# Graph-COM/HEPT

Measured on AMD Instinct MI355X. Metric: attention-fwd points/sec, higher is better.
Workload: dtype bf16

## Files before the change

### hept_amd/csrc/block_attn.hip

```cpp
#include "common.h"
#include "p2p_dev.h"

namespace {

#ifndef HEPT_ATTN_STORE
#define HEPT_ATTN_STORE 1
#endif
__device__ __forceinline__ void store16_rows(unsigned int* dst, const u32x4& v) {
#if HEPT_ATTN_STORE == 1
    __builtin_nontemporal_store(v, reinterpret_cast<u32x4*>(dst));
#else
    *reinterpret_cast<u32x4*>(dst) = v;
#endif
}

#ifndef HEPT_RAGGED16_WAVES
#define HEPT_RAGGED16_WAVES 7
#endif
constexpr int attn_waves(int nkt, bool bf16, bool p16, bool full, bool diff = false) {
    if (diff) return full ? 3 : 2;
    return bf16 ? ((nkt == 3 && !p16 && full) ? 6 : (full ? 8 : HEPT_RAGGED16_WAVES)) : (full ? 6 : 4);
}
template <int NKT, bool BF16, bool P16, bool F16QK, bool FULL, bool DIFF = false>
__global__ __launch_bounds__(64 * NKT) __attribute__((amdgpu_waves_per_eu(attn_waves(NKT, BF16, P16, FULL, DIFF), attn_waves(NKT, BF16, P16, FULL, DIFF))))
void block_attn_kernel(const char* __restrict__ qhat,
                                                              const char* __restrict__ kvhat,
                                                              const int* __restrict__ qpos,
                                                              const int* __restrict__ kpos,
                                                              float* __restrict__ part, int N, int H, int D, int B,
                                                              int nb, HeadRange hr, PushArgs pa) {
    if (pa.push_wgs > 0 && (int)blockIdx.x < pa.push_wgs) {
        reduce_push_body<P16>(pa, (int)blockIdx.x);
        return;
    }
    constexpr int NT = 64 * NKT;
    constexpr int KEYS = 32 * NKT;
    constexpr int ESZ = BF16 ? 2 : 4;
    constexpr int QROW = 32 * ESZ;
    constexpr int KVROW = 2 * QROW;
    constexpr int CH = QROW / 16;
    constexpr int CPR = 2 * CH;

    extern __shared__ __attribute__((aligned(16))) char smem[];
    char* k_s = smem;
    char* v_s = smem + KEYS * QROW;
    float* kn_s = reinterpret_cast<float*>(smem + 2 * KEYS * QROW);
    int* qidx_s = reinterpret_cast<int*>(smem + 2 * KEYS * QROW + KEYS * 4);

    const int tid = threadIdx.x, lane = tid & 63, w = tid >> 6, hh = lane >> 5, li = lane & 31;
    const int bid = (int)blockIdx.x - pa.push_wgs;
    const int h = hr.h0 + bid % hr.hg;
    const int rest = bid / hr.hg;
    const int b = hr.tl > 0 ? rest / hr.tl : rest % nb, t = hr.tl > 0 ? rest % hr.tl : rest / nb;
    const size_t seg = ((size_t)t * H + h) * N + (size_t)b * B;
    const int* __restrict__ kp = kpos + seg;
    const int* __restrict__ qp = qpos + seg;
    const char* __restrict__ qbase = qhat + (size_t)h * N * QROW;
    const char* __restrict__ kvbase = kvhat + (size_t)h * N * KVROW;

    const int qi = w * 32 + li;
    const bool qvalid = FULL || qi < B;
    const int qsrc = qp[qvalid ? qi : 0];
    if (hh == 0) qidx_s[qi] = qvalid ? qsrc : -1;
    const char* qrow = qbase + (size_t)qsrc * QROW;
    float qn = *reinterpret_cast<const float*>(qrow + QROW - 4);
    u32x4 qraw[BF16 ? 2 : 4];
#pragma unroll
    for (int s = 0; s < (BF16 ? 2 : 4); ++s)
        qraw[s] = *reinterpret_cast<const u32x4*>(qrow + (BF16 ? (s * 32 + hh * 16) : (hh * 64 + s * 16)));
    if (hh == 1) qraw[BF16 ? 1 : 3][3] = 0u;
    if constexpr (DIFF) {
        static_assert(!BF16, "the difference form runs on f32 rows");
        float part = 0.f;
#pragma unroll
        for (int s2 = 0; s2 < 4; ++s2)
#pragma unroll
            for (int j = 0; j < 4; ++j) {
                const bool feat = 16 * hh + 4 * s2 + j < D;
                const float qv = __uint_as_float(qraw[s2][j]);
                part = feat ? fmaf(qv, qv, part) : part;
                if (!feat) qraw[s2][j] = 0u;
            }
        qn = -0.5f * (part + __shfl_xor(part, 32));
    }

#pragma unroll
    for (int it = 0; it < CPR / 2; ++it) {
        const int ci = it * NT + tid;
        const int key = ci / CPR, c = ci % CPR;
        u32x4 val = {0u, 0u, 0u, 0u};
        if (FULL || key < B) {
            const int src = kp[key];
            val = *reinterpret_cast<const u32x4*>(kvbase + (size_t)src * KVROW + c * 16);
        }
        if (c < CH) {
            if (c == CH - 1) {
                kn_s[key] = __uint_as_float(val[3]);
                val[3] = 0u;
            }
            const int sw = BF16 ? ((key >> 2) & 3) : ((key >> 1) & 7);
            *reinterpret_cast<u32x4*>(k_s + key * QROW + ((c ^ sw) * 16)) = val;
        } else {
            *reinterpret_cast<u32x4*>(v_s + key * QROW + (c - CH) * 16) = val;
        }
    }
    __syncthreads();
    if constexpr (DIFF) {
        if (tid < KEYS) {
            const int sw = (tid >> 1) & 7;
            float acc = 0.f;
            for (int col = 0; col < D; ++col) {
                const float kv2 = *reinterpret_cast<const float*>(k_s + tid * QROW + (((col >> 2) ^ sw) * 16) + (col & 3) * 4);
                acc = fmaf(kv2, kv2, acc);
            }
            kn_s[tid] = -0.5f * acc;
        }
        __syncthreads();
    }

    f32x16 z;
#pragma unroll
    for (int r = 0; r < 16; ++r) z[r] = 0.f;

#pragma unroll
    for (int kt = 0; kt < NKT; ++kt) {
        if (!FULL && kt * 32 >= B) break;
        const int key = kt * 32 + li;
        f32x16 x;
#pragma unroll
        for (int r = 0; r < 16; ++r) x[r] = qn + kn_s[kt * 32 + hept_acc_row(r, hh)];

        if constexpr (BF16) {
#pragma unroll
            for (int s = 0; s < 2; ++s) {
                const int c = 2 * s + hh;
                const u32x4 kraw =
                    *reinterpret_cast<const u32x4*>(k_s + key * QROW + ((c ^ ((key >> 2) & 3)) * 16));
                if constexpr (F16QK)
                    x = __builtin_amdgcn_mfma_f32_32x32x16_f16(__builtin_bit_cast(f16x8, kraw),
                                                               __builtin_bit_cast(f16x8, qraw[s]), x, 0, 0, 0);
                else
                    x = __builtin_amdgcn_mfma_f32_32x32x16_bf16(__builtin_bit_cast(bf16x8, kraw),
                                                                __builtin_bit_cast(bf16x8, qraw[s]), x, 0, 0, 0);
            }
        } else {
            float kf[16];
#pragma unroll
            for (int c = 0; c < 4; ++c) {
                const f32x4 kk = *reinterpret_cast<const f32x4*>(
                    k_s + key * QROW + (((4 * hh + c) ^ ((key >> 1) & 7)) * 16));
                kf[4 * c] = kk[0]; kf[4 * c + 1] = kk[1]; kf[4 * c + 2] = kk[2]; kf[4 * c + 3] = kk[3];
            }
#pragma unroll
            for (int s = 0; s < 16; ++s)
                x = __builtin_amdgcn_mfma_f32_32x32x2f32(kf[s], __uint_as_float(qraw[s >> 2][s & 3]), x, 0, 0, 0);
            if constexpr (DIFF) {
                float dsq[16];
#pragma unroll
                for (int r = 0; r < 16; ++r) dsq[r] = 0.f;
                for (int col = D; col < 30; ++col) {
                    const float qc = *reinterpret_cast<const float*>(qrow + col * 4);
#pragma unroll
                    for (int r = 0; r < 16; ++r) {
                        const int kr = kt * 32 + hept_acc_row(r, hh);
                        const float kc = *reinterpret_cast<const float*>(
                            k_s + kr * QROW + (((col >> 2) ^ ((kr >> 1) & 7)) * 16) + (col & 3) * 4);
                        const float dlt = qc - kc;
                        dsq[r] = fmaf(dlt, dlt, dsq[r]);
                    }
                }
#pragma unroll
                for (int r = 0; r < 16; ++r) x[r] = fmaf(-0.5f, dsq[r], x[r]);
            }
        }

        float pr[16];
        exp_clamped(x, pr);
        if (!FULL && (kt + 1) * 32 > B) {
#pragma unroll
            for (int r = 0; r < 16; ++r)
                if (kt * 32 + hept_acc_row(r, hh) >= B) pr[r] = 0.f;
        }

        if constexpr (BF16) {
            const int g = lane >> 4, l16 = lane & 15;
            const int vrow = kt * 32 + 4 * hh + (l16 >> 2);
            const int vcol = 32 * (g & 1) + 8 * (l16 & 3);
#pragma unroll
            for (int s = 0; s < 2; ++s) {
                u32x4 pw;
#pragma unroll
                for (int j = 0; j < 4; ++j) pw[j] = hept_pack_bf16(pr[8 * s + 2 * j], pr[8 * s + 2 * j + 1]);
                const s16x4 v0 = __builtin_amdgcn_ds_read_tr16_b64_v4i16(
                    (lds_s16x4_ptr)(v_s + (vrow + 16 * s) * QROW + vcol));
                const s16x4 v1 = __builtin_amdgcn_ds_read_tr16_b64_v4i16(
                    (lds_s16x4_ptr)(v_s + (vrow + 16 * s + 8) * QROW + vcol));
                typedef __attribute__((ext_vector_type(8))) short s16x8;
                const s16x8 vv = {v0[0], v0[1], v0[2], v0[3], v1[0], v1[1], v1[2], v1[3]};
                z = __builtin_amdgcn_mfma_f32_32x32x16_bf16(__builtin_bit_cast(bf16x8, pw),
                                                            __builtin_bit_cast(bf16x8, vv), z, 0, 0, 0);
            }
        } else {
#pragma unroll
            for (int r = 0; r < 16; ++r) {
                const float vv =
                    *reinterpret_cast<const float*>(v_s + (kt * 32 + hept_acc_row(r, hh)) * QROW + li * 4);
                z = __builtin_amdgcn_mfma_f32_32x32x2f32(pr[r], vv, z, 0, 0, 0);
            }
        }
    }

    if constexpr (P16) {
        __syncthreads();
        float* tile = reinterpret_cast<float*>(smem) + w * 32 * 32;
        {
            float* wr = tile + (4 * hh) * 32 + li;
#pragma unroll
            for (int r = 0; r < 16; ++r) wr[((r & 3) + 8 * (r >> 2)) * 32] = z[r];
        }
        unsigned int* __restrict__ pt =
            reinterpret_cast<unsigned int*>(part) + (size_t)t * hr.tstride_rows * 16 + (size_t)(h - hr.hsub) * 16;
#pragma unroll
        for (int j = 0; j < 2; ++j) {
            const int row = (lane >> 2) + 16 * j, pc = lane & 3;
            const int q2 = w * 32 + row;
            const f32x4 f0 = *reinterpret_cast<const f32x4*>(tile + row * 32 + pc * 8);
            const f32x4 f1 = *reinterpret_cast<const f32x4*>(tile + row * 32 + pc * 8 + 4);
            u32x4 v = {hept_pack_bf16(f0[0], f0[1]), hept_pack_bf16(f0[2], f0[3]), hept_pack_bf16(f1[0], f1[1]),
                       hept_pack_bf16(f1[2], f1[3])};
            if (pc == 3) v = u32x4{__float_as_uint(f0[0] + 1e-20f), 0u, 0u, 0u};
            if (FULL || q2 < B) {
                const int dst = qidx_s[q2];
                if (pa.direct) {
                    bool remote;
                    char* rowp = direct_row(pa, dst, h - hr.h0, 64, remote) + pc * 16;
                    if (remote) store16_system(rowp, v);
                    else *reinterpret_cast<u32x4*>(rowp) = v;
                } else {
                    store16_rows(pt + (size_t)dst * hr.hout * 16 + pc * 4, v);
                }
            }
        }
    } else {
        float* __restrict__ pt = part + (size_t)t * hr.tstride_rows * 32 + (size_t)(h - hr.hsub) * 32 + li;
#pragma unroll
        for (int r = 0; r < 16; ++r) {
            const int q2 = w * 32 + hept_acc_row(r, hh);
            if (FULL || q2 < B) {
                const int dst = qidx_s[q2];
                float val = z[r];
                if (li == D) val += 1e-20f;
                if (pa.direct) {
                    bool remote;
                    char* rowp = direct_row(pa, dst, h - hr.h0, 128, remote) + li * 4;
                    if (remote) store4_system(rowp, __float_as_uint(val));
                    else *reinterpret_cast<float*>(rowp) = val;
                } else {
                    pt[(size_t)dst * hr.hout * 32] = val;
                }
            }
        }
    }
    if (pa.direct) {
        drain_remote_stores();
        if (pa.counter) signal_when_all_done(pa.counter, pa.peers, pa.world, pa.flag_idx, pa.epoch, gridDim.x - pa.push_wgs);
    }
}

#ifndef HEPT_SPLIT_CK8
#define HEPT_SPLIT_CK8 128
#endif
constexpr int split_ck(int nkt) { return nkt == 8 ? HEPT_SPLIT_CK8 : (nkt >= 2 ? 64 : 32); }
#ifndef HEPT_SPLIT_PP
#define HEPT_SPLIT_PP 2
#endif
template <int NKT, bool FULL, int VP, bool DIFF = false>
__global__ __launch_bounds__(64 * NKT) void block_attn_split_kernel(const float* __restrict__ qhat,
                                                                    const float* __restrict__ kvhat,
                                                                    const int* __restrict__ qpos,
                                                                    const int* __restrict__ kpos,
                                                                    float* __restrict__ part, int N, int H, int D,
                                                                    int B, int nb, HeadRange hr, PushArgs pa) {
    if (pa.push_wgs > 0 && (int)blockIdx.x < pa.push_wgs) {
        reduce_push_body<false>(pa, (int)blockIdx.x);
        return;
    }
    constexpr int NT = 64 * NKT;
    constexpr int KEYS = 32 * NKT;
    constexpr int PROW = 64;
    constexpr int CK = split_ck(NKT);
    constexpr int NCH = (KEYS + CK - 1) / CK;
    constexpr int IPT = (CK * 8 + NT - 1) / NT;
    extern __shared__ __attribute__((aligned(16))) char smem[];
    char* k_s = smem;
    char* v_s = smem + 3 * CK * PROW;
    float* kc_s = reinterpret_cast<float*>(smem + (3 + VP) * CK * PROW);

    const int tid = threadIdx.x, lane = tid & 63, w = tid >> 6, hh = lane >> 5, li = lane & 31;
    const int bid = (int)blockIdx.x - pa.push_wgs;
    const int h = hr.h0 + bid % hr.hg;
    const int rest = bid / hr.hg;
    const int b = hr.tl > 0 ? rest / hr.tl : rest % nb, t = hr.tl > 0 ? rest % hr.tl : rest / nb;
    const size_t seg = ((size_t)t * H + h) * N + (size_t)b * B;
    const int* __restrict__ kp = kpos + seg;
    const int* __restrict__ qp = qpos + seg;
    const float* __restrict__ qbase = qhat + (size_t)h * N * 32;
    const float* __restrict__ kvbase = kvhat + (size_t)h * N * 64;

    float pre[IPT][8];
    auto fetch = [&](int ch) {
#pragma unroll
        for (int it = 0; it < IPT; ++it) {
            const int ci = it * NT + tid;
            const int key = ch * CK + (ci >> 3), c = ci & 7;
#pragma unroll
            for (int j = 0; j < 8; ++j) pre[it][j] = 0.f;
            if (ci < CK * 8 && key < (FULL ? KEYS : B)) {
                const int ks = kp[key];
                if (c >= 4 && hr.vsrc) {
                    const int col = 8 * (c - 4);
                    const float* src = hr.vsrc + ((size_t)ks * H + h) * D + col;
                    const bool real = ks < hr.raw_size;
                    if (real && col < D) {
                        const f32x4 a0 = *reinterpret_cast<const f32x4*>(src);
                        pre[it][0] = a0[0]; pre[it][1] = a0[1]; pre[it][2] = a0[2]; pre[it][3] = a0[3];
                    }
                    if (real && col + 4 < D) {
                        const f32x4 a1 = *reinterpret_cast<const f32x4*>(src + 4);
                        pre[it][4] = a1[0]; pre[it][5] = a1[1]; pre[it][6] = a1[2]; pre[it][7] = a1[3];
                    }
                    if (col == D) pre[it][0] = 1.f;
                    if (col + 4 == D) pre[it][4] = 1.f;
                } else {
                    const float* src = kvbase + (size_t)ks * 64 + c * 8;
                    const f32x4 a0 = *reinterpret_cast<const f32x4*>(src);
                    const f32x4 a1 = *reinterpret_cast<const f32x4*>(src + 4);
                    pre[it][0] = a0[0]; pre[it][1] = a0[1]; pre[it][2] = a0[2]; pre[it][3] = a0[3];
                    pre[it][4] = a1[0]; pre[it][5] = a1[1]; pre[it][6] = a1[2]; pre[it][7] = a1[3];
                    if (c == 3) pre[it][6] = 1.f;
                }
            }
        }
    };
    auto stage = [&]() {
#pragma unroll
        for (int it = 0; it < IPT; ++it) {
            const int ci = it * NT + tid;
            if (ci >= CK * 8) break;
            const int row = ci >> 3, c = ci & 7;
            u32x4 ph, pm, pl;
            if constexpr (DIFF) {
                float sq = 0.f;
                if (c < 3) {
#pragma unroll
                    for (int j = 0; j < 8; ++j) sq = fmaf(pre[it][j], pre[it][j], sq);
                }
                const int sqi = __builtin_bit_cast(int, sq);
                const float s1 = __builtin_bit_cast(float, __builtin_amdgcn_update_dpp(0, sqi, 0x111, 0xF, 0xF, true));
                const float s2 = __builtin_bit_cast(float, __builtin_amdgcn_update_dpp(0, sqi, 0x112, 0xF, 0xF, true));
                const float s3 = __builtin_bit_cast(float, __builtin_amdgcn_update_dpp(0, sqi, 0x113, 0xF, 0xF, true));
                if (c == 3) {
                    *reinterpret_cast<f32x4*>(kc_s + row * 8) = f32x4{pre[it][0], pre[it][1], pre[it][2], pre[it][3]};
                    *reinterpret_cast<f32x4*>(kc_s + row * 8 + 4) = f32x4{pre[it][4], pre[it][5], 0.f, 0.f};
#pragma unroll
                    for (int j = 0; j < 6; ++j) pre[it][j] = 0.f;
                    pre[it][7] = -0.5f * ((s3 + s2) + s1);
                }
            }
            if (c < 4) {
                split3_bf16(pre[it], ph, pm, pl);
                const int off = row * PROW + ((c ^ ((row >> 2) & 3)) * 16);
                *reinterpret_cast<u32x4*>(k_s + off) = ph;
                *reinterpret_cast<u32x4*>(k_s + CK * PROW + off) = pm;
                *reinterpret_cast<u32x4*>(k_s + 2 * CK * PROW + off) = pl;
            } else {
                if constexpr (VP == 3) split3_bf16(pre[it], ph, pm, pl);
                else split2_bf16(pre[it], ph, pm);
                const int off = row * PROW + (c - 4) * 16;
                *reinterpret_cast<u32x4*>(v_s + off) = ph;
                *reinterpret_cast<u32x4*>(v_s + CK * PROW + off) = pm;
                if constexpr (VP == 3) *reinterpret_cast<u32x4*>(v_s + 2 * CK * PROW + off) = pl;
            }
        }
    };
    fetch(0);

    const int qi = w * 32 + li;
    const bool qvalid = FULL || qi < B;
    const int qsrc = qp[qvalid ? qi : 0];
    const float* qrow = qbase + (size_t)qsrc * 32;
    u32x4 qh[2], qm[2], ql[2];
    float qc[DIFF ? 6 : 1];
    {
        float av[2][8];
#pragma unroll
        for (int s = 0; s < 2; ++s) {
            const f32x4 a0 = *reinterpret_cast<const f32x4*>(qrow + 16 * s + 8 * hh);
            const f32x4 a1 = *reinterpret_cast<const f32x4*>(qrow + 16 * s + 8 * hh + 4);
            av[s][0] = a0[0]; av[s][1] = a0[1]; av[s][2] = a0[2]; av[s][3] = a0[3];
            av[s][4] = a1[0]; av[s][5] = a1[1]; av[s][6] = a1[2]; av[s][7] = a1[3];
        }
        if constexpr (DIFF) {
            float fn = 0.f;
#pragma unroll
            for (int j = 0; j < 8; ++j) fn = fmaf(av[0][j], av[0][j], fn);
            if (hh == 0) {
#pragma unroll
                for (int j = 0; j < 8; ++j) fn = fmaf(av[1][j], av[1][j], fn);
            }
            fn += __shfl_xor(fn, 32);
#pragma unroll
            for (int c = 0; c < 6; ++c) qc[c] = __shfl(av[1][c], li + 32);
            if (hh == 1) {
#pragma unroll
                for (int j = 0; j < 6; ++j) av[1][j] = 0.f;
                av[1][6] = -0.5f * fn;
                av[1][7] = 1.f;
            }
        } else if (hh == 1) {
            av[1][6] = av[1][7];
            av[1][7] = 1.f;
        }
#pragma unroll
        for (int s = 0; s < 2; ++s) split3_bf16(av[s], qh[s], qm[s], ql[s]);
    }

    f32x16 z;
#pragma unroll
    for (int r = 0; r < 16; ++r) z[r] = 0.f;
    const int krow[2] = {li * PROW + ((hh ^ ((li >> 2) & 3)) * 16), li * PROW + (((2 + hh) ^ ((li >> 2) & 3)) * 16)};
    const int vlane = (4 * hh + ((lane & 15) >> 2)) * PROW + 32 * ((lane >> 4) & 1) + 8 * (lane & 3);

#pragma unroll
    for (int ch = 0; ch < NCH; ++ch) {
        if (!FULL && ch * CK >= B) break;
        if (ch > 0) __syncthreads();
        stage();
        if (ch + 1 < NCH) fetch(ch + 1);
        __syncthreads();
        constexpr int TPC = CK / 32, GRP = TPC < 2 ? TPC : 2;
#pragma unroll
        for (int g0 = 0; g0 < TPC; g0 += GRP) {
        f32x16 xs[GRP];
#pragma unroll
        for (int kg = 0; kg < GRP; ++kg) {
            const int kl = g0 + kg;
            const int kt = ch * TPC + kl;
            if (kt >= NKT) break;
            if (!FULL && kt * 32 >= B) break;
#pragma unroll
            for (int r = 0; r < 16; ++r) xs[kg][r] = 0.f;
#pragma unroll
            for (int s = 0; s < 2; ++s) {
                const int off = kl * 32 * PROW + krow[s];
                const u32x4 kh = *reinterpret_cast<const u32x4*>(k_s + off);
                const u32x4 km = *reinterpret_cast<const u32x4*>(k_s + CK * PROW + off);
                const u32x4 kl3 = *reinterpret_cast<const u32x4*>(k_s + 2 * CK * PROW + off);
                xs[kg] = mfma_bf16(kl3, qh[s], xs[kg]);
                xs[kg] = mfma_bf16(kh, ql[s], xs[kg]);
                xs[kg] = mfma_bf16(km, qm[s], xs[kg]);
                xs[kg] = mfma_bf16(km, qh[s], xs[kg]);
                xs[kg] = mfma_bf16(kh, qm[s], xs[kg]);
                xs[kg] = mfma_bf16(kh, qh[s], xs[kg]);
            }
        }
#pragma unroll
        for (int kg = 0; kg < GRP; ++kg) {
            const int kl = g0 + kg;
            const int kt = ch * TPC + kl;
            if (kt >= NKT) break;
            if (!FULL && kt * 32 >= B) break;
            f32x16 x = xs[kg];
            if constexpr (DIFF) {
#pragma unroll
                for (int r = 0; r < 16; ++r) {
                    const float* kc = kc_s + (kl * 32 + hept_acc_row(r, hh)) * 8;
                    const f32x4 k0 = *reinterpret_cast<const f32x4*>(kc), k1 = *reinterpret_cast<const f32x4*>(kc + 4);
                    float d0 = qc[0] - k0[0], d1 = qc[1] - k0[1], d2 = qc[2] - k0[2], d3 = qc[3] - k0[3];
                    float d4 = qc[4] - k1[0], d5 = qc[5] - k1[1];
                    float dsq = d0 * d0;
                    dsq = fmaf(d1, d1, dsq); dsq = fmaf(d2, d2, dsq); dsq = fmaf(d3, d3, dsq);
                    dsq = fmaf(d4, d4, dsq); dsq = fmaf(d5, d5, dsq);
                    x[r] = fmaf(-0.5f, dsq, x[r]);
                }
            }

            float pr[16];
            exp_clamped(x, pr);
            if (!FULL && (kt + 1) * 32 > B) {
#pragma unroll
                for (int r = 0; r < 16; ++r)
                    if (kt * 32 + hept_acc_row(r, hh) >= B) pr[r] = 0.f;
            }

#pragma unroll
            for (int s = 0; s < 2; ++s) {
                float pa[8];
#pragma unroll
                for (int j = 0; j < 8; ++j) pa[j] = pr[8 * s + j];
                constexpr int PP = HEPT_SPLIT_PP;
                u32x4 pp[3];
                if constexpr (PP == 3) split3_bf16(pa, pp[0], pp[1], pp[2]);
                else split2_bf16(pa, pp[0], pp[1]);
                typedef __attribute__((ext_vector_type(8))) short s16x8;
                u32x4 vpl[VP];
#pragma unroll
                for (int pl = 0; pl < VP; ++pl) {
                    const char* vb = v_s + pl * CK * PROW + (kl * 32 + 16 * s) * PROW + vlane;
                    const s16x4 v0 = __builtin_amdgcn_ds_read_tr16_b64_v4i16((lds_s16x4_ptr)(vb));
                    const s16x4 v1 = __builtin_amdgcn_ds_read_tr16_b64_v4i16((lds_s16x4_ptr)(vb + 8 * PROW));
                    const s16x8 vv = {v0[0], v0[1], v0[2], v0[3], v1[0], v1[1], v1[2], v1[3]};
                    vpl[pl] = __builtin_bit_cast(u32x4, vv);
                }
#pragma unroll
                for (int ord = 2; ord >= 0; --ord)
#pragma unroll
                    for (int i = PP - 1; i >= 0; --i) {
                        const int j = ord - i;
                        if (j >= 0 && j < VP) z = mfma_bf16(pp[i], vpl[j], z);
                    }
            }
        }
        }
    }

    __syncthreads();
    float* tile = reinterpret_cast<float*>(smem) + w * 32 * 32;
    {
        float* wr = tile + (4 * hh) * 32 + li;
#pragma unroll
        for (int r = 0; r < 16; ++r) wr[((r & 3) + 8 * (r >> 2)) * 32] = z[r];
    }
    float* __restrict__ pt = part + (size_t)t * hr.tstride_rows * 32 + (size_t)(h - hr.hsub) * 32;
#pragma unroll
    for (int j = 0; j < 4; ++j) {
        const int row = (lane >> 3) + 8 * j, pc = lane & 7;
        const int q2 = w * 32 + row;
        const int dst = __shfl(qsrc, row);
        f32x4 f = *reinterpret_cast<const f32x4*>(tile + row * 32 + pc * 4);
#pragma unroll
        for (int e = 0; e < 4; ++e)
            if (pc * 4 + e == D) f[e] += 1e-20f;
        if (FULL || q2 < B) {
            if (pa.direct) {
                bool remote;
                char* rowp = direct_row(pa, dst, h - hr.h0, 128, remote) + pc * 16;
                if (remote) store16_system(rowp, __builtin_bit_cast(u32x4, f));
                else *reinterpret_cast<f32x4*>(rowp) = f;
            } else {
                *reinterpret_cast<f32x4*>(pt + (size_t)dst * hr.hout * 32 + pc * 4) = f;
            }
        }
    }
    if (pa.direct) {
        drain_remote_stores();
        if (pa.counter) signal_when_all_done(pa.counter, pa.peers, pa.world, pa.flag_idx, pa.epoch, gridDim.x - pa.push_wgs);
    }
}

template <bool FULL, int VP, bool DIFF = false>
int launch_attn_split(int nkt, dim3 grid, hipStream_t st, const float* qhat, const float* kvhat, const int* qpos,
                      const int* kpos, float* part, int N, int H, int D, int B, int nb, HeadRange hr, PushArgs pa) {
#define HEPT_SPLIT_CASE(K)                                                                                       \
    case K: {                                                                                                    \
                          \
        constexpr size_t lds0 = (size_t)(3 + VP) * split_ck(K) * 64 + (DIFF ? (size_t)split_ck(K) * 32 : 0);        \
        constexpr size_t lds = lds0 > (size_t)K * 4096 ? lds0 : (size_t)K * 4096;                                \
        if (lds > 65536) {                                                                                       \
            static LdsRaised raised;                                                                             \
            if (hept_raise_lds(raised, reinterpret_cast<const void*>(&block_attn_split_kernel<K, FULL, VP, DIFF>), lds)) \
                return HEPT_ERR_LAUNCH;                                                                          \
        }                                                                                                        \
        hipLaunchKernelGGL((block_attn_split_kernel<K, FULL, VP, DIFF>), grid, dim3(64 * K), lds, st, qhat, kvhat, qpos, \
                           kpos, part, N, H, D, B, nb, hr, pa);                                                        \
        break;                                                                                                   \
    }
    switch (nkt) {
        HEPT_SPLIT_CASE(1)
        HEPT_SPLIT_CASE(2)
        HEPT_SPLIT_CASE(3)
        HEPT_SPLIT_CASE(4)
        HEPT_SPLIT_CASE(5)
        HEPT_SPLIT_CASE(6)
        HEPT_SPLIT_CASE(7)
        HEPT_SPLIT_CASE(8)
        default:
            return HEPT_ERR_SHAPE;
    }
#undef HEPT_SPLIT_CASE
    return hept_launch_status();
}

template <bool BF16, bool P16, bool F16QK, bool FULL, bool DIFF = false>
int launch_attn_full(int nkt, dim3 grid, hipStream_t st, const char* qhat, const char* kvhat, const int* qpos,
                const int* kpos, float* part, int N, int H, int D, int B, int nb, HeadRange hr, PushArgs pa) {
#define HEPT_ATTN_CASE(K)                                                                                    \
    case K: {                                                                                                \
        constexpr size_t lds = (size_t)2 * 32 * K * 32 * (BF16 ? 2 : 4) + 32 * K * 8;                        \
        if (lds > 65536) {                                                                                   \
            static LdsRaised raised;                                                                         \
            if (hept_raise_lds(raised, reinterpret_cast<const void*>(&block_attn_kernel<K, BF16, P16, F16QK, FULL, DIFF>), lds)) \
                return HEPT_ERR_LAUNCH;                                                                      \
        }                                                                                                    \
        hipLaunchKernelGGL((block_attn_kernel<K, BF16, P16, F16QK, FULL, DIFF>), grid, dim3(64 * K), lds, st, qhat, kvhat, qpos, \
                           kpos, part, N, H, D, B, nb, hr, pa);                                                    \
        break;                                                                                               \
    }
    switch (nkt) {
        HEPT_ATTN_CASE(1)
        HEPT_ATTN_CASE(2)
        HEPT_ATTN_CASE(3)
        HEPT_ATTN_CASE(4)
        HEPT_ATTN_CASE(5)
        HEPT_ATTN_CASE(6)
        HEPT_ATTN_CASE(7)
        HEPT_ATTN_CASE(8)
        default:
            return HEPT_ERR_SHAPE;
    }
#undef HEPT_ATTN_CASE
    return hept_launch_status();
}

template <bool BF16, bool P16, bool F16QK, bool DIFF = false>
int launch_attn(int nkt, dim3 grid, hipStream_t st, const char* qhat, const char* kvhat, const int* qpos,
                const int* kpos, float* part, int N, int H, int D, int B, int nb, HeadRange hr, PushArgs pa) {
    if (B == 32 * nkt)
        return launch_attn_full<BF16, P16, F16QK, true, DIFF>(nkt, grid, st, qhat, kvhat, qpos, kpos, part, N, H, D, B, nb, hr, pa);
    return launch_attn_full<BF16, P16, F16QK, false, DIFF>(nkt, grid, st, qhat, kvhat, qpos, kpos, part, N, H, D, B, nb, hr, pa);
}

}

namespace {
int block_attn_impl(const void* qhat, const void* kvhat, const int32_t* qpos, const int32_t* kpos, int N, int H, int D,
                    int Tl, int B, int precision, const HeadRange& hr_in, float* part, void* stream,
                    const PushArgs* push = nullptr, VSrc vs = VSrc{}) {
    HeadRange hr = hr_in;
    hr.vsrc = nullptr;
    hr.raw_size = N;
    static const bool table_major = [] { const char* e = getenv("HEPT_ATTN_TABLE_MAJOR"); return e && *e && *e != '0'; }();
    hr.tl = table_major ? 0 : Tl;
    if (vs.v) {
        if (precision != HEPT_PREC_F32 || D % 4 != 0 || (reinterpret_cast<uintptr_t>(vs.v) & 15)) return HEPT_ERR_ARG;
        hr.vsrc = vs.v;
        hr.raw_size = vs.raw_size;
    }
    if (!qhat || !kvhat || !qpos || !kpos || (!part && !(push && push->direct))) return HEPT_ERR_ARG;
    if (N < 1 || H < 1 || Tl < 1 || B < 1 || B > HEPT_MAX_BLOCK || N % B != 0 || D < 1 || D > 28)
        return HEPT_ERR_SHAPE;
    if (hr.h0 < 0 || hr.hg < 1 || hr.h0 + hr.hg > H || hr.hout < 1 || hr.hsub < 0 || hr.hsub > hr.h0 ||
        hr.h0 + hr.hg - hr.hsub > hr.hout)
        return HEPT_ERR_SHAPE;

    const int nb = N / B, nkt = (B + 31) / 32;
    PushArgs pa{};
    if (push) {
        pa = *push;
        if (pa.direct ? (pa.push_wgs != 0 || Tl != 1 || pa.h0 != hr.h0 || pa.hg != hr.hg) : pa.push_wgs < 1)
            return HEPT_ERR_ARG;
    }
    const dim3 grid((unsigned)((size_t)Tl * nb * hr.hg + pa.push_wgs));
    hipStream_t st = (hipStream_t)stream;
    const char* qh = (const char*)qhat;
    const char* kv = (const char*)kvhat;
    if (precision == HEPT_PREC_BF16 && D == 24)
        return launch_attn<true, true, false>(nkt, grid, st, qh, kv, qpos, kpos, part, N, H, D, B, nb, hr, pa);
    if (precision == HEPT_PREC_BF16)
        return launch_attn<true, false, false>(nkt, grid, st, qh, kv, qpos, kpos, part, N, H, D, B, nb, hr, pa);
    if (precision == HEPT_PREC_MIXED16 && D == 24)
        return launch_attn<true, true, true>(nkt, grid, st, qh, kv, qpos, kpos, part, N, H, D, B, nb, hr, pa);
    if (precision == HEPT_PREC_MIXED16)
        return launch_attn<true, false, true>(nkt, grid, st, qh, kv, qpos, kpos, part, N, H, D, B, nb, hr, pa);
    if (precision == HEPT_PREC_F32) {
        const float* qf = (const float*)qhat;
        const float* kf = (const float*)kvhat;
        if (B == 32 * nkt) return launch_attn_split<true, 3>(nkt, grid, st, qf, kf, qpos, kpos, part, N, H, D, B, nb, hr, pa);
        return launch_attn_split<false, 3>(nkt, grid, st, qf, kf, qpos, kpos, part, N, H, D, B, nb, hr, pa);
    }
    if (precision == HEPT_PREC_F32_MFMA)
        return launch_attn<false, false, false>(nkt, grid, st, qh, kv, qpos, kpos, part, N, H, D, B, nb, hr, pa);
    if (precision == HEPT_PREC_F32_DIFF) {
        const char* e = getenv("HEPT_DIFF_MFMA");
        const bool mfma = e && *e && *e != '0';
        if (D == 24 && !mfma) {
            const float* qf = (const float*)qhat;
            const float* kf = (const float*)kvhat;
            if (B == 32 * nkt) return launch_attn_split<true, 3, true>(nkt, grid, st, qf, kf, qpos, kpos, part, N, H, D, B, nb, hr, pa);
            return launch_attn_split<false, 3, true>(nkt, grid, st, qf, kf, qpos, kpos, part, N, H, D, B, nb, hr, pa);
        }
        return launch_attn<false, false, false, true>(nkt, grid, st, qh, kv, qpos, kpos, part, N, H, D, B, nb, hr, pa);
    }
    return HEPT_ERR_SHAPE;
}
}

int hept_block_attn_heads_push(const void* qhat, const void* kvhat, const int32_t* qpos, const int32_t* kpos, int N,
                               int H, int D, int Tl, int B, int precision, int h0, int hg, int hout, int hsub,
                               int n_rows_out, float* part, const PushArgs* push, void* stream, VSrc vs) {
    if (n_rows_out < N) return HEPT_ERR_SHAPE;
    const HeadRange hr{h0, hg, hout, hsub, (long long)n_rows_out * hout, nullptr, 0, 0};
    return block_attn_impl(qhat, kvhat, qpos, kpos, N, H, D, Tl, B, precision, hr, part, stream, push, vs);
}

extern "C" int hept_block_attn(const void* qhat, const void* kvhat, const int32_t* qpos, const int32_t* kpos, int N,
                               int H, int D, int Tl, int B, int precision, float* part, void* stream) {
    const HeadRange all{0, H, H, 0, (long long)N * H, nullptr, 0, 0};
    return block_attn_impl(qhat, kvhat, qpos, kpos, N, H, D, Tl, B, precision, all, part, stream);
}

extern "C" int hept_block_attn_heads(const void* qhat, const void* kvhat, const int32_t* qpos, const int32_t* kpos,
                                     int N, int H, int D, int Tl, int B, int precision, int h0, int hg, int hout,
                                     int hsub, int n_rows_out, float* part, void* stream) {
    if (n_rows_out < N) return HEPT_ERR_SHAPE;
    const HeadRange hr{h0, hg, hout, hsub, (long long)n_rows_out * hout, nullptr, 0, 0};
    return block_attn_impl(qhat, kvhat, qpos, kpos, N, H, D, Tl, B, precision, hr, part, stream);
}
```

### hept_amd/csrc/common.h

```cpp
#pragma once
#include <hip/hip_runtime.h>
#include <stdint.h>
#include "../../include/hept_hip.h"

#define HEPT_WAVE 64

typedef __attribute__((ext_vector_type(4))) float f32x4;
typedef __attribute__((ext_vector_type(16))) float f32x16;
typedef __attribute__((ext_vector_type(8))) __bf16 bf16x8;
typedef __attribute__((ext_vector_type(4))) short s16x4;
typedef __attribute__((ext_vector_type(4))) unsigned int u32x4;

struct HeadRange {
    int h0, hg, hout, hsub;
    long long tstride_rows;
    const float* vsrc;
    int raw_size;
    int tl;
};
struct VSrc {
    const float* v = nullptr;
    int raw_size = 0;
};

static inline bool hept_f32_rows(int precision) {
    return precision == HEPT_PREC_F32 || precision == HEPT_PREC_F32_MFMA || precision == HEPT_PREC_F32_DIFF;
}

static inline int hept_launch_status() {
    hipError_t e = hipGetLastError();
    return e == hipSuccess ? HEPT_OK : HEPT_ERR_LAUNCH;
}

#define HEPT_MAX_DEVICES 64
struct LdsRaised {
    bool done[HEPT_MAX_DEVICES] = {};
};
static inline int hept_raise_lds(LdsRaised& flags, const void* fn, size_t bytes) {
    int dev = 0;
    if (hipGetDevice(&dev) != hipSuccess || dev < 0 || dev >= HEPT_MAX_DEVICES) return HEPT_ERR_LAUNCH;
    if (flags.done[dev]) return HEPT_OK;
    if (hipFuncSetAttribute(fn, hipFuncAttributeMaxDynamicSharedMemorySize, (int)bytes) != hipSuccess) return HEPT_ERR_LAUNCH;
    flags.done[dev] = true;
    return HEPT_OK;
}

#define HEPT_FSUM_OUT 16
#define HEPT_FSUM_SLICES 16
__device__ __forceinline__ float hept_fixed_sum(const float* __restrict__ partial, int n_parts, size_t pitch, int o,
                                               bool valid, float* red_s ) {
    const int ol = threadIdx.x % HEPT_FSUM_OUT, sl = threadIdx.x / HEPT_FSUM_OUT;
    float acc = 0.f;
    if (valid)
        for (int g = sl; g < n_parts; g += HEPT_FSUM_SLICES) acc += partial[(size_t)g * pitch + o];
    red_s[sl * HEPT_FSUM_OUT + ol] = acc;
    __syncthreads();
    float tot = 0.f;
    if (sl == 0)
        for (int s2 = 0; s2 < HEPT_FSUM_SLICES; ++s2) tot += red_s[s2 * HEPT_FSUM_OUT + ol];
    return tot;
}

typedef __attribute__((ext_vector_type(2))) float hept_f32x2;
typedef __attribute__((ext_vector_type(2))) __bf16 hept_bf16x2;
__device__ __forceinline__ unsigned int hept_pack_bf16(float lo, float hi) {
    const hept_f32x2 v = {lo, hi};
    return __builtin_bit_cast(unsigned int, __builtin_convertvector(v, hept_bf16x2));
}
__device__ __forceinline__ float hept_bf16_lo(unsigned int w) { return __uint_as_float(w << 16); }
__device__ __forceinline__ float hept_bf16_hi(unsigned int w) { return __uint_as_float(w & 0xFFFF0000u); }

typedef __attribute__((ext_vector_type(2))) _Float16 hept_f16x2;
typedef __attribute__((ext_vector_type(8))) _Float16 f16x8;
__device__ __forceinline__ unsigned int hept_pack_f16(float lo, float hi) {
    const hept_f32x2 v = {fminf(fmaxf(lo, -65504.f), 65504.f), fminf(fmaxf(hi, -65504.f), 65504.f)};
    return __builtin_bit_cast(unsigned int, __builtin_convertvector(v, hept_f16x2));
}
__device__ __forceinline__ unsigned int hept_pack_f16_ieee(float lo, float hi) {
    const hept_f32x2 v = {lo, hi};
    return __builtin_bit_cast(unsigned int, __builtin_convertvector(v, hept_f16x2));
}
__device__ __forceinline__ float hept_f16_lo(unsigned int w) { return (float)__builtin_bit_cast(hept_f16x2, w)[0]; }
__device__ __forceinline__ float hept_f16_hi(unsigned int w) { return (float)__builtin_bit_cast(hept_f16x2, w)[1]; }

typedef __attribute__((ext_vector_type(2))) unsigned int u32x2;
template <int IN>
__device__ __forceinline__ float hept_in_lo(unsigned int w) {
    if constexpr (IN == HEPT_IN_BF16) return hept_bf16_lo(w);
    else return hept_f16_lo(w);
}
template <int IN>
__device__ __forceinline__ float hept_in_hi(unsigned int w) {
    if constexpr (IN == HEPT_IN_BF16) return hept_bf16_hi(w);
    else return hept_f16_hi(w);
}
template <int IN>
__device__ __forceinline__ f32x4 hept_widen4(unsigned int w0, unsigned int w1) {
    return f32x4{hept_in_lo<IN>(w0), hept_in_hi<IN>(w0), hept_in_lo<IN>(w1), hept_in_hi<IN>(w1)};
}
template <int IN>
__device__ __forceinline__ unsigned int hept_narrow2(float lo, float hi) {
    if constexpr (IN == HEPT_IN_BF16) return hept_pack_bf16(lo, hi);
    else return hept_pack_f16_ieee(lo, hi);
}
template <int IN>
__device__ __forceinline__ float hept_in_elem(const void* x, size_t i) {
    if constexpr (IN == HEPT_IN_F32) return reinterpret_cast<const float*>(x)[i];
    else return hept_in_lo<IN>(reinterpret_cast<const unsigned short*>(x)[i]);
}

__device__ __forceinline__ int hept_acc_row(int r, int hh) { return (r & 3) + 8 * (r >> 2) + 4 * hh; }

typedef s16x4 __attribute__((address_space(3))) * lds_s16x4_ptr;
__device__ __forceinline__ void split3_bf16(const float (&a)[8], u32x4& h, u32x4& m, u32x4& l) {
#pragma unroll
    for (int j = 0; j < 4; ++j) {
        const unsigned int hp = hept_pack_bf16(a[2 * j], a[2 * j + 1]);
        const float r0 = a[2 * j] - hept_bf16_lo(hp), r1 = a[2 * j + 1] - hept_bf16_hi(hp);
        const unsigned int mp = hept_pack_bf16(r0, r1);
        const float s0 = r0 - hept_bf16_lo(mp), s1 = r1 - hept_bf16_hi(mp);
        h[j] = hp;
        m[j] = mp;
        l[j] = hept_pack_bf16(s0, s1);
    }
}
__device__ __forceinline__ void split2_bf16(const float (&a)[8], u32x4& h, u32x4& m) {
#pragma unroll
    for (int j = 0; j < 4; ++j) {
        const unsigned int hp = hept_pack_bf16(a[2 * j], a[2 * j + 1]);
        h[j] = hp;
        m[j] = hept_pack_bf16(a[2 * j] - hept_bf16_lo(hp), a[2 * j + 1] - hept_bf16_hi(hp));
    }
}
__device__ __forceinline__ f32x16 mfma_bf16(const u32x4& a, const u32x4& b, f32x16 c) {
    return __builtin_amdgcn_mfma_f32_32x32x16_bf16(__builtin_bit_cast(bf16x8, a), __builtin_bit_cast(bf16x8, b), c, 0,
                                                   0, 0);
}

__device__ __forceinline__ void exp_clamped(const f32x16& x, float (&pr)[16]) {
    typedef __attribute__((ext_vector_type(2))) float f32x2_t;
#pragma unroll
    for (int j = 0; j < 8; ++j) {
        const f32x2_t t = f32x2_t{x[2 * j], x[2 * j + 1]} * f32x2_t{1.442695041f, 1.442695041f};
        pr[2 * j] = __builtin_fminf(__builtin_fmaxf(__builtin_amdgcn_exp2f(t[0]), 0.f), 1.f);
        pr[2 * j + 1] = __builtin_fminf(__builtin_fmaxf(__builtin_amdgcn_exp2f(t[1]), 0.f), 1.f);
    }
}

#ifndef HEPT_NT_PREP_IN
#define HEPT_NT_PREP_IN 1
#endif
#ifndef HEPT_NT_KA_IN
#define HEPT_NT_KA_IN 1
#endif
#ifndef HEPT_NT_KB_IN
#define HEPT_NT_KB_IN 1
#endif
#ifndef HEPT_NT_RIDER_IN32
#define HEPT_NT_RIDER_IN32 1
#endif
#ifndef HEPT_NT_RIDER_IN16
#define HEPT_NT_RIDER_IN16 0
#endif
#ifndef HEPT_NT_CODES
#define HEPT_NT_CODES 0
#endif
#ifndef HEPT_NT_OUT
#define HEPT_NT_OUT 0
#endif
#ifndef HEPT_NT_BWD_ROWS
#define HEPT_NT_BWD_ROWS 0
#endif
template <bool NT, typename T>
__device__ __forceinline__ T hept_ld(const T* p) {
    if constexpr (NT) return __builtin_nontemporal_load(p);
    else return *p;
}
template <bool NT, typename T>
__device__ __forceinline__ void hept_st(T* p, const T& v) {
    if constexpr (NT) __builtin_nontemporal_store(v, p);
    else *p = v;
}

__device__ __forceinline__ unsigned int hept_wave_scan_add(unsigned int x) {
    x += (unsigned int)__builtin_amdgcn_update_dpp(0, (int)x, 0x111, 0xF, 0xF, true);
    x += (unsigned int)__builtin_amdgcn_update_dpp(0, (int)x, 0x112, 0xF, 0xF, true);
    x += (unsigned int)__builtin_amdgcn_update_dpp(0, (int)x, 0x114, 0xF, 0xF, true);
    x += (unsigned int)__builtin_amdgcn_update_dpp(0, (int)x, 0x118, 0xF, 0xF, true);
    x += (unsigned int)__builtin_amdgcn_update_dpp(0, (int)x, 0x142, 0xA, 0xF, true);
    x += (unsigned int)__builtin_amdgcn_update_dpp(0, (int)x, 0x143, 0xC, 0xF, true);
    return x;
}
__device__ __forceinline__ unsigned int hept_wave_sum(unsigned int x) {
    return (unsigned int)__builtin_amdgcn_readlane((int)hept_wave_scan_add(x), 63);
}
__device__ __forceinline__ unsigned int hept_wave_max(unsigned int x) {
    auto mx = [](unsigned int a, unsigned int b) { return a > b ? a : b; };
    x = mx(x, (unsigned int)__builtin_amdgcn_update_dpp(0, (int)x, 0x111, 0xF, 0xF, true));
    x = mx(x, (unsigned int)__builtin_amdgcn_update_dpp(0, (int)x, 0x112, 0xF, 0xF, true));
    x = mx(x, (unsigned int)__builtin_amdgcn_update_dpp(0, (int)x, 0x114, 0xF, 0xF, true));
    x = mx(x, (unsigned int)__builtin_amdgcn_update_dpp(0, (int)x, 0x118, 0xF, 0xF, true));
    x = mx(x, (unsigned int)__builtin_amdgcn_update_dpp(0, (int)x, 0x142, 0xA, 0xF, true));
    x = mx(x, (unsigned int)__builtin_amdgcn_update_dpp(0, (int)x, 0x143, 0xC, 0xF, true));
    return (unsigned int)__builtin_amdgcn_readlane((int)x, 63);
}

int hept_prep_hash_rpe(const void* q, const void* k, const void* v, const float* coords, const float* sqrt_w, int K,
                       const float* alpha, const int64_t* codes, int N, int raw_size, int H, int D, int C, int T, int t0,
                       int Tl, int precision, void* qhat, void* kvhat, float* qproj, float* kproj, float* minmax,
                       void* stream, int roles = 3,
                       void* zero_ptr = nullptr, size_t zero_bytes = 0,
                       int in_dtype = HEPT_IN_F32);
int hept_prep_hash_fused_rpe(const void* x, int io_dtype, int ldx, const float* norm_w, const float* norm_b, float eps, const float* w_q,
                             const float* w_k, const float* w_v, const float* coords, const float* sqrt_w, int K,
                             const float* alpha, const int64_t* codes, int N, int raw_size, int H, int D, int C, int T,
                             int t0, int Tl, int precision, void* qhat, void* kvhat, float* qproj, float* kproj,
                             float* minmax, void* stream, void* zero_ptr = nullptr, size_t zero_bytes = 0);
int hept_combine_ffn_ld(const float* part, int part_precision, int Tl, int N, int H, int D, int n0, int n_count,
                        const float* out_weight, const float* out_bias, const void* x, int io_dtype, int ldx,
                        const float* norm_w, const float* norm_b, float eps, const float* ff1_w, const float* ff1_b,
                        const float* ff2_w, const float* ff2_b, void* y, int ldy, void* stream);
struct HeptRowsJob {
    const void* v;
    void* kvhat;
    int N, raw_size, H, D, precision;
    int in_dtype;
};
bool hept_sort_carries_rows(int N, int H, int D);
int hept_sort_tables_rows(const float* qproj, const float* kproj, const int64_t* codes, const float* minmax, int N, int H,
                          int T, int t0, int Tl, void* sort_ws, int32_t* qpos, int32_t* kpos, const HeptRowsJob* rows,
                          void* stream, bool zeroed = false);
int hept_sort_tables_src_rows(const float* qproj, const float* kproj, const float* eta_idx, const float* phi_idx,
                              const float* cfac, float* minmax, int N, int H, int T, int t0, int Tl, void* sort_ws,
                              int32_t* qpos, int32_t* kpos, const HeptRowsJob* rows, void* stream, bool zeroed = false);
void hept_sort_zero_block(void* sort_ws, int N, int H, int Tl, void** ptr, size_t* bytes);
void hept_prof_mark_sort_mid(void* stream);
int hept_segmented_argsort_bounded(const float* keys, int S, int L, float lo, float hi, void* ws, int32_t* pos,
                                   void* stream);
```

Baseline: 384.1 million.

## Use 3D grid indexing and batch K/V staging loads with early index prefetch

Replaces the 1D grid's div/mod decoding of head, batch-block and time indices with a 3D grid, falling back to linear indexing when dimensions exceed limits. Push-reduction workgroups are placed in extra z-slices, and any surplus slots go idle. The K/V staging loop is restructured so each thread loads its key indices early and stages a fixed column, with a configurable number of loads in flight. An optional direct global-to-LDS load path is added behind a flag that is off by default. The intent is to cut integer index math and expose more memory parallelism during staging, at the cost of idle padding workgroups and more complex dispatch logic.

```diff
diff --git a/hept_amd/csrc/block_attn.hip b/hept_amd/csrc/block_attn.hip
--- a/hept_amd/csrc/block_attn.hip
+++ b/hept_amd/csrc/block_attn.hip
@@ -14,6 +14,38 @@
 #endif
 }
 
+constexpr int ATTN_WG = -1, ATTN_IDLE = -2;
+__device__ __forceinline__ int attn_workgroup(const HeadRange& hr, const PushArgs& pa, int nb, int& h, int& t, int& b) {
+    int bx = (int)blockIdx.x, by = (int)blockIdx.y, bz = (int)blockIdx.z;
+    if (hr.zpush | hr.lin) {
+        if (hr.lin) {
+            const int bid = bx - pa.push_wgs;
+            if (bid < 0) return bx;
+            bx = bid % hr.hg;
+            const int rest = bid / hr.hg, inner = hr.tl > 0 ? hr.tl : nb;
+            by = rest % inner;
+            bz = rest / inner;
+        } else {
+            const int lin = bx + (int)gridDim.x * (by + (int)gridDim.y * bz);
+            if (lin < pa.push_wgs) return lin;
+            if (bz < hr.zpush) return ATTN_IDLE;
+            bz -= hr.zpush;
+        }
+    }
+    h = hr.h0 + bx;
+    t = hr.tl > 0 ? by : bz;
+    b = hr.tl > 0 ? bz : by;
+    return ATTN_WG;
+}
+__device__ __forceinline__ unsigned int attn_workgroups() { return gridDim.x * gridDim.y * gridDim.z; }
+
+#ifndef HEPT_ATTN_LDS_DMA
+#define HEPT_ATTN_LDS_DMA 0
+#endif
+#ifndef HEPT_ATTN_STAGE_INFLIGHT
+#define HEPT_ATTN_STAGE_INFLIGHT 1
+#endif
+
 #ifndef HEPT_RAGGED16_WAVES
 #define HEPT_RAGGED16_WAVES 7
 #endif
@@ -29,8 +61,10 @@
                                                               const int* __restrict__ kpos,
                                                               float* __restrict__ part, int N, int H, int D, int B,
                                                               int nb, HeadRange hr, PushArgs pa) {
-    if (pa.push_wgs > 0 && (int)blockIdx.x < pa.push_wgs) {
-        reduce_push_body<P16>(pa, (int)blockIdx.x);
+    int h, t, b;
+    const int wg = attn_workgroup(hr, pa, nb, h, t, b);
+    if (wg != ATTN_WG) {
+        if (wg >= 0) reduce_push_body<P16>(pa, wg);
         return;
     }
     constexpr int NT = 64 * NKT;
@@ -48,10 +82,6 @@
     int* qidx_s = reinterpret_cast<int*>(smem + 2 * KEYS * QROW + KEYS * 4);
 
     const int tid = threadIdx.x, lane = tid & 63, w = tid >> 6, hh = lane >> 5, li = lane & 31;
-    const int bid = (int)blockIdx.x - pa.push_wgs;
-    const int h = hr.h0 + bid % hr.hg;
-    const int rest = bid / hr.hg;
-    const int b = hr.tl > 0 ? rest / hr.tl : rest % nb, t = hr.tl > 0 ? rest % hr.tl : rest / nb;
     const size_t seg = ((size_t)t * H + h) * N + (size_t)b * B;
     const int* __restrict__ kp = kpos + seg;
     const int* __restrict__ qp = qpos + seg;
@@ -61,7 +91,18 @@
     const int qi = w * 32 + li;
     const bool qvalid = FULL || qi < B;
     const int qsrc = qp[qvalid ? qi : 0];
-    if (hh == 0) qidx_s[qi] = qvalid ? qsrc : -1;
+    constexpr int KPI = NT / CPR, SITS = CPR / 2, SGRP = HEPT_ATTN_STAGE_INFLIGHT;
+    static_assert(SGRP == 1 || SGRP == 2 || SGRP == 4, "HEPT_ATTN_STAGE_INFLIGHT");
+    constexpr bool DMA = HEPT_ATTN_LDS_DMA && BF16 && FULL;
+    const int sc = tid % CPR, skey0 = tid / CPR;
+    int ksrc[SGRP];
+    if constexpr (!DMA) {
+#pragma unroll
+        for (int j = 0; j < SGRP; ++j) {
+            const int key = j * KPI + skey0;
+            ksrc[j] = (FULL || key < B) ? kp[key] : 0;
+        }
+    }
     const char* qrow = qbase + (size_t)qsrc * QROW;
     float qn = *reinterpret_cast<const float*>(qrow + QROW - 4);
     u32x4 qraw[BF16 ? 2 : 4];
@@ -84,26 +125,58 @@
         qn = -0.5f * (part + __shfl_xor(part, 32));
     }
 
-#pragma unroll
-    for (int it = 0; it < CPR / 2; ++it) {
-        const int ci = it * NT + tid;
-        const int key = ci / CPR, c = ci % CPR;
-        u32x4 val = {0u, 0u, 0u, 0u};
-        if (FULL || key < B) {
+    if constexpr (DMA) {
+#pragma unroll
+        for (int i = 0; i < 4; ++i) {
+            const int blk = i * NKT + w;
+            const int key = (blk - (i >= 2 ? 2 * NKT : 0)) * 16 + (lane >> 2), p = lane & 3;
+            const int c = i >= 2 ? CH + p : (p ^ ((key >> 2) & 3));
             const int src = kp[key];
-            val = *reinterpret_cast<const u32x4*>(kvbase + (size_t)src * KVROW + c * 16);
-        }
-        if (c < CH) {
-            if (c == CH - 1) {
-                kn_s[key] = __uint_as_float(val[3]);
-                val[3] = 0u;
-            }
-            const int sw = BF16 ? ((key >> 2) & 3) : ((key >> 1) & 7);
-            *reinterpret_cast<u32x4*>(k_s + key * QROW + ((c ^ sw) * 16)) = val;
-        } else {
-            *reinterpret_cast<u32x4*>(v_s + key * QROW + (c - CH) * 16) = val;
-        }
-    }
+            __builtin_amdgcn_global_load_lds(
+                (const __attribute__((address_space(1))) void*)(kvbase + (size_t)src * KVROW + c * 16),
+                (__attribute__((address_space(3))) void*)(smem + blk * 1024), 16, 0, 0);
+        }
+        asm volatile("s_waitcnt vmcnt(0)" ::: "memory");
+#pragma unroll
+        for (int i = 0; i < 2; ++i) {
+            const int blk = i * NKT + w;
+            const int key = blk * 16 + (lane >> 2), p = lane & 3;
+            if ((p ^ ((key >> 2) & 3)) == CH - 1) {
+                unsigned int* nw = reinterpret_cast<unsigned int*>(smem + blk * 1024 + lane * 16 + 12);
+                kn_s[key] = __uint_as_float(*nw);
+                *nw = 0u;
+            }
+        }
+    } else {
+        const bool nrm = sc == CH - 1;
+#pragma unroll
+        for (int g0 = 0; g0 < SITS; g0 += SGRP) {
+            if (g0 > 0) {
+#pragma unroll
+                for (int j = 0; j < SGRP; ++j) {
+                    const int key = (g0 + j) * KPI + skey0;
+                    ksrc[j] = (FULL || key < B) ? kp[key] : 0;
+                }
+            }
+            u32x4 val[SGRP];
+#pragma unroll
+            for (int j = 0; j < SGRP; ++j) {
+                const int key = (g0 + j) * KPI + skey0;
+                val[j] = u32x4{0u, 0u, 0u, 0u};
+                if (FULL || key < B) val[j] = *reinterpret_cast<const u32x4*>(kvbase + (size_t)ksrc[j] * KVROW + sc * 16);
+            }
+#pragma unroll
+            for (int j = 0; j < SGRP; ++j) {
+                const int key = (g0 + j) * KPI + skey0;
+                if (nrm) kn_s[key] = __uint_as_float(val[j][3]);
+                val[j][3] = nrm ? 0u : val[j][3];
+                const int sw = BF16 ? ((key >> 2) & 3) : ((key >> 1) & 7);
+                const int off = sc < CH ? ((sc ^ sw) * 16) : (KEYS * QROW + (sc - CH) * 16);
+                *reinterpret_cast<u32x4*>(smem + key * QROW + off) = val[j];
+            }
+        }
+    }
+    if (hh == 0) qidx_s[qi] = qvalid ? qsrc : -1;
     __syncthreads();
     if constexpr (DIFF) {
         if (tid < KEYS) {
@@ -263,7 +336,7 @@
     }
     if (pa.direct) {
         drain_remote_stores();
-        if (pa.counter) signal_when_all_done(pa.counter, pa.peers, pa.world, pa.flag_idx, pa.epoch, gridDim.x - pa.push_wgs);
+        if (pa.counter) signal_when_all_done(pa.counter, pa.peers, pa.world, pa.flag_idx, pa.epoch, attn_workgroups());
     }
 }
 
@@ -281,8 +354,10 @@
                                                                     const int* __restrict__ kpos,
                                                                     float* __restrict__ part, int N, int H, int D,
                                                                     int B, int nb, HeadRange hr, PushArgs pa) {
-    if (pa.push_wgs > 0 && (int)blockIdx.x < pa.push_wgs) {
-        reduce_push_body<false>(pa, (int)blockIdx.x);
+    int h, t, b;
+    const int wg = attn_workgroup(hr, pa, nb, h, t, b);
+    if (wg != ATTN_WG) {
+        if (wg >= 0) reduce_push_body<false>(pa, wg);
         return;
     }
     constexpr int NT = 64 * NKT;
@@ -297,10 +372,6 @@
     float* kc_s = reinterpret_cast<float*>(smem + (3 + VP) * CK * PROW);
 
     const int tid = threadIdx.x, lane = tid & 63, w = tid >> 6, hh = lane >> 5, li = lane & 31;
-    const int bid = (int)blockIdx.x - pa.push_wgs;
-    const int h = hr.h0 + bid % hr.hg;
-    const int rest = bid / hr.hg;
-    const int b = hr.tl > 0 ? rest / hr.tl : rest % nb, t = hr.tl > 0 ? rest % hr.tl : rest / nb;
     const size_t seg = ((size_t)t * H + h) * N + (size_t)b * B;
     const int* __restrict__ kp = kpos + seg;
     const int* __restrict__ qp = qpos + seg;
@@ -554,7 +625,7 @@
     }
     if (pa.direct) {
         drain_remote_stores();
-        if (pa.counter) signal_when_all_done(pa.counter, pa.peers, pa.world, pa.flag_idx, pa.epoch, gridDim.x - pa.push_wgs);
+        if (pa.counter) signal_when_all_done(pa.counter, pa.peers, pa.world, pa.flag_idx, pa.epoch, attn_workgroups());
     }
 }
 
@@ -660,7 +731,12 @@
         if (pa.direct ? (pa.push_wgs != 0 || Tl != 1 || pa.h0 != hr.h0 || pa.hg != hr.hg) : pa.push_wgs < 1)
             return HEPT_ERR_ARG;
     }
-    const dim3 grid((unsigned)((size_t)Tl * nb * hr.hg + pa.push_wgs));
+    const int gy = hr.tl > 0 ? Tl : nb, gz = hr.tl > 0 ? nb : Tl;
+    hr.zpush = (int)(((size_t)pa.push_wgs + (size_t)hr.hg * gy - 1) / ((size_t)hr.hg * gy));
+    hr.lin = gy > 65535 || (long long)gz + hr.zpush > 65535;
+    if (hr.lin) hr.zpush = 0;
+    const dim3 grid = hr.lin ? dim3((unsigned)((size_t)Tl * nb * hr.hg + pa.push_wgs))
+                             : dim3((unsigned)hr.hg, (unsigned)gy, (unsigned)(gz + hr.zpush));
     hipStream_t st = (hipStream_t)stream;
     const char* qh = (const char*)qhat;
     const char* kv = (const char*)kvhat;
diff --git a/hept_amd/csrc/common.h b/hept_amd/csrc/common.h
--- a/hept_amd/csrc/common.h
+++ b/hept_amd/csrc/common.h
@@ -17,6 +17,7 @@
     const float* vsrc;
     int raw_size;
     int tl;
+    int zpush, lin;
 };
 struct VSrc {
     const float* v = nullptr;
```

Measured after the change: 391.0 million (median of 4 runs). 1.8% higher.
